# isl-org/Open3D-ML

Hardware: NVIDIA H100
Metric: M points/s forward (higher is better)
Workload: dtype f32

## Files before the change

include/o3dml_b200.h:

```cpp
#ifndef O3DML_B200_H
#define O3DML_B200_H

#include <stddef.h>
#include <stdint.h>

#ifdef __cplusplus
extern "C" {
#endif

#define O3DML_ABI_VERSION 2
#define O3DML_API __attribute__((visibility("default")))

#define O3DML_ACT_NONE 0
#define O3DML_ACT_RELU 1
#define O3DML_ACT_LEAKY 2

O3DML_API int o3dml_abi_version(void);
O3DML_API const char* o3dml_last_error(void);
O3DML_API unsigned long long o3dml_launch_count(void);
O3DML_API void o3dml_launch_count_add(unsigned long long n);


O3DML_API size_t o3dml_voxelize_workspace_bytes(int64_t num_points, int64_t batch);
O3DML_API int o3dml_voxelize(const float* points, int64_t num_points, int point_stride,
// ... 127 lines not shown
                                    const void* weight_image, int k_pad, int n_pad, const float* scale,
                                    const float* shift, int act, float slope, float* out,
                                    int out_channels, void* stream);
O3DML_API int o3dml_deconv_nhwc_tc(const float* in, int batch, int H, int W, int C, int stride,
                                   const void* weight_image, int k_pad, int n_pad, const float* scale,
                                   const float* shift, int act, float slope, float* out, int out_ld,
                                   int out_channels, void* stream);

O3DML_API int o3dml_linear_rows_small_supported(int channels0, int channels1, int out_channels);
O3DML_API int o3dml_linear_rows_small(int64_t num_rows, const o3dml_src_t* srcs, int num_srcs,
                                      const float* h_weight_t, const float* h_scale,
                                      const float* h_shift, int act, float slope, float* out, int out_ld,
                                      int out_channels, void* stream);


O3DML_API int o3dml_randla_lfa_pool(int stage, int d, const float* coords, const void* neighbor_idx,
                          int idx_is64, int num_neighbors, const float* feat, int64_t batch,
                          int64_t n_per_batch, const float* w10_t, const float* s10,
                          const float* t10, const float* wl2_t, const float* s2, const float* t2,
                          const float* wscore_t, const float* bscore, float* agg, void* stream);

#define O3DML_LFA16_WEIGHT_FLOATS 448
O3DML_API int o3dml_randla_lfa16_pool(int stage, const float* coords, const void* neighbor_idx, int idx_is64,
                                      int num_neighbors, const float* feat, int64_t batch,
                                      int64_t n_per_batch, const float* h_weights, float* agg,
                                      void* stream);

O3DML_API int o3dml_randla_lfa_pool_tc(int stage, int d, const float* coords, const void* neighbor_idx,
                                       int idx_is64, int num_neighbors, const float* feat, int64_t batch,
                                       int64_t n_per_batch, const float* w10_t, const float* s10,
                                       const float* t10, const void* wl2_image, const float* wl2_t,
                                       const float* s2, const float* t2, const void* wscore_image,
                                       float* agg, void* stream);

O3DML_API int o3dml_randla_tail_supported(int skip_channels, int coarse_channels, int c1, int c2, int c3, int classes);
O3DML_API int o3dml_randla_tail(const float* skip, int skip_ld, const float* coarse, int coarse_ld,
                                int64_t coarse_rows, const void* interp_index, int index_is64,
                                int64_t out_rows_per_batch, int64_t src_rows_per_batch, int64_t num_rows,
                                const void* weight_image, const float* h_scale, const float* h_shift, float slope,
                                int classes, float* out, void* stream);

O3DML_API int o3dml_gather_max(const float* src, int64_t src_rows, int channels, int src_ld,
                     const void* index, int index_is64, int64_t num_rows, int k,
                     int64_t out_rows_per_batch, int64_t src_rows_per_batch, int shadow_zero,
                     float* out, int out_ld, void* stream);


O3DML_API int o3dml_kpconv_gather(const float* query_points, int64_t num_queries,
                        const float* support_points, int64_t num_support,
                        const void* neighbor_index, int index_is64, int max_neighbors,
                        const float* features, int in_channels, const float* kernel_points,
                        int num_kernel_points, float kp_extent, float* weighted_features,
                        void* stream);

O3DML_API int o3dml_kpconv_gather_deformable(const float* query_points, int64_t num_queries,
                        const float* support_points, int64_t num_support,
                        const void* neighbor_index, int index_is64, int max_neighbors,
                        const float* features, int in_channels, const float* kernel_points,
                        int num_kernel_points, float kp_extent, const float* offsets, int offset_ld,
                        float* weighted_features, void* stream);

#ifdef __cplusplus
}
#endif
#endif
```

open3d-ml_b200/_lib.py:

```python
import ctypes
import math
import os

import torch

_HERE = os.path.dirname(os.path.abspath(__file__))
LIB_PATH = os.path.join(_HERE, "lib", "libo3dml_b200.so")
_lib = None
ABI_VERSION = 2

c_void_p, c_int, c_int64, c_float, c_size_t = (ctypes.c_void_p, ctypes.c_int, ctypes.c_int64,
                                               ctypes.c_float, ctypes.c_size_t)


class Src(ctypes.Structure):
    _fields_ = [("data", c_void_p), ("index", c_void_p), ("rows", c_int64),
                ("out_rows_per_batch", c_int64), ("src_rows_per_batch", c_int64),
                ("channels", ctypes.c_int32), ("ld", ctypes.c_int32),
                ("index_is64", ctypes.c_int32), ("index_ld", ctypes.c_int32)]


P, I, L, F, Z = c_void_p, c_int, c_int64, c_float, c_size_t
_SIGNATURES = {
    "o3dml_abi_version": (c_int, []),
# ... 4 lines not shown
    "o3dml_voxelize": (I, [P, L, I, P, L, P, P, P, L, L, P, P, P, P, P, P, P, Z, P]),
    "o3dml_ragged_to_dense": (I, [P, I, L, P, L, L, L, L, P, P]),
    "o3dml_knn_workspace_bytes": (Z, [L, L, L]),
    "o3dml_knn_search": (I, [P, L, P, P, L, P, L, I, P, I, P, P, Z, P]),
    "o3dml_radius_workspace_bytes": (Z, [L, L, L]),
    "o3dml_radius_count": (I, [P, L, P, P, L, P, L, F, P, P, P, Z, P]),
    "o3dml_radius_fill": (I, [P, L, L, P, L, F, P, P, P, P, Z, P]),
    "o3dml_voxel_reduce": (I, [P, I, P, I, I, P, P, P, P, L, I, I, P, P, P, P]),
    "o3dml_reduce_subarrays_sum": (I, [P, P, L, P, P]),
    "o3dml_sparse_conv_workspace_bytes": (Z, [L]),
    "o3dml_sparse_conv_neighbors": (I, [P, L, P, L, F, P, P, I, P, P, P, Z, P]),
    "o3dml_continuous_conv": (I, [P, I, I, I, I, I, P, L, P, I, P, P, P, L, P, P, I, P, P, I, I, I, I, P, P]),
    "o3dml_nms_workspace_bytes": (Z, [L]),
    "o3dml_nms": (I, [P, P, L, F, P, P, P, Z, P]),
    "o3dml_iou_matrix": (I, [P, L, P, L, I, P, P]),
    "o3dml_pp_detect_workspace_bytes": (Z, [L, L, L, I, I, L]),
    "o3dml_pp_detect": (I, [P, L, P, L, P, L, L, L, L, I, I, P, L, F, F, P, P, P, P, P, Z, P]),
    "o3dml_pp_pfn_scatter": (I, [P, I, I, P, P, P, P, P, L, P, P, P, I, F, F, F, F, I, I, I, P, P,
                                 I, P]),
    "o3dml_pp_pfn2_scatter": (I, [P, I, I, P, P, P, P, P, L, P, P, P, P, P, P, I, F, F, F, F, I, I, I, P, P,
                                  I, P]),
    "o3dml_linear": (I, [L, ctypes.POINTER(Src), I, P, P, P, P, I, I, F, P, I, I, I, P]),
    "o3dml_conv3x3_nhwc": (I, [P, I, I, I, I, I, P, P, P, I, F, P, I, P]),
    "o3dml_deconv_nhwc": (I, [P, I, I, I, I, I, P, P, P, I, F, P, I, I, P]),
    "o3dml_linear_tc_supported": (I, [ctypes.POINTER(Src), I]),
    "o3dml_linear_tc": (I, [L, ctypes.POINTER(Src), I, P, I, I, P, P, P, I, I, F, P, I, I, I, P]),
    "o3dml_conv3x3_nhwc_tc": (I, [P, I, I, I, I, I, P, I, I, P, P, I, F, P, I, P]),
    "o3dml_deconv_nhwc_tc": (I, [P, I, I, I, I, I, P, I, I, P, P, I, F, P, I, I, P]),
    "o3dml_randla_lfa_pool": (I, [I, I, P, P, I, I, P, L, L, P, P, P, P, P, P, P, P, P, P]),
    "o3dml_linear_rows_small_supported": (I, [I, I, I]),
    "o3dml_linear_rows_small": (I, [L, P, I, P, P, P, I, F, P, I, I, P]),
    "o3dml_randla_lfa16_pool": (I, [I, P, P, I, I, P, L, L, P, P, P]),
    "o3dml_randla_lfa_pool_tc": (I, [I, I, P, P, I, I, P, L, L, P, P, P, P, P, P, P, P, P, P]),
    "o3dml_randla_tail_supported": (I, [I, I, I, I, I, I]),
    "o3dml_randla_tail": (I, [P, I, P, I, L, P, I, L, L, L, P, P, P, F, I, P, P]),
    "o3dml_gather_max": (I, [P, L, I, I, P, I, L, I, L, L, I, P, I, P]),
    "o3dml_kpconv_gather": (I, [P, L, P, L, P, I, I, P, I, P, I, F, P, P]),
    "o3dml_kpconv_gather_deformable": (I, [P, L, P, L, P, I, I, P, I, P, I, F, P, I, P, P]),
}
EXPORTS = tuple(_SIGNATURES)
_BRINGUP_SIGNATURES = {
    "o3dml_tc_gemm_test": (I, [P, P, P, I, I, I, P]),
    "o3dml_tc_mma_rate": (I, [I, I, P, P]),
}


def lib():
    global _lib
    if _lib is None:
        from . import build as _build
        have_nvcc = os.path.exists(_build.NVCC)
        if have_nvcc or not os.path.exists(LIB_PATH):
            try:
                _build.build()
            except Exception as e:
                if not os.path.exists(LIB_PATH):
                    raise RuntimeError(
                        "open3d_ml_b200: CUDA library %s is missing and could not be built (%s). "
                        "There is no CPU fallback." % (LIB_PATH, e)) from e
                raise
        h = ctypes.CDLL(LIB_PATH)
        for name, (res, args) in list(_SIGNATURES.items()) + list(_BRINGUP_SIGNATURES.items()):
            fn = getattr(h, name)
            fn.restype, fn.argtypes = res, args
        if h.o3dml_abi_version() != ABI_VERSION:
            raise RuntimeError("open3d_ml_b200: ABI version mismatch")
# ... 235 lines not shown
```

open3d-ml_b200/csrc/common.cuh:

```cuda
#pragma once
#include <cuda_runtime.h>
#include <stdint.h>
#include <stdio.h>
#include <atomic>
#include <utility>

#define O3DML_OK 0
#define O3DML_ERR_INVALID 1
#define O3DML_ERR_WORKSPACE 2
#define O3DML_ERR_CUDA 3
#define O3DML_ERR_UNSUPPORTED 4

extern "C" void o3dml_set_error(const char* fmt, ...);

#define O3DML_FAIL(code, ...)      \
    do {                           \
        o3dml_set_error(__VA_ARGS__); \
        return (code);             \
    } while (0)

#define O3DML_CHECK(cond, ...)                               \
    do {                                                     \
        if (!(cond)) O3DML_FAIL(O3DML_ERR_INVALID, __VA_ARGS__); \
    } while (0)

#define O3DML_CHECK_WORKSPACE(ws, entry)                                                                    \
    do {                                                                                                    \
        if (!(ws).ok) O3DML_FAIL(O3DML_ERR_WORKSPACE, entry ": workspace too small (%zu needed)", (ws).off); \
    } while (0)

#define O3DML_CUDA(...)                                                               \
    do {                                                                              \
        cudaError_t e__ = (__VA_ARGS__);                                              \
        if (e__ != cudaSuccess)                                                       \
            O3DML_FAIL(O3DML_ERR_CUDA, "%s failed: %s (%s:%d)", #__VA_ARGS__,         \
                       cudaGetErrorString(e__), __FILE__, __LINE__);                  \
    } while (0)

namespace o3dml {

constexpr int kNumSMs = 132;

void count_launch();

template <auto Kernel>
cudaError_t opt_in_smem(size_t smem) {
    if (smem <= 48 * 1024) return cudaSuccess;
    static std::atomic<unsigned long long> done{0};
    int dev = -1;
    if (cudaGetDevice(&dev) != cudaSuccess || dev >= 64) dev = -1;
    if (dev >= 0 && ((done.load(std::memory_order_relaxed) >> dev) & 1ull)) return cudaSuccess;
    const cudaError_t e = cudaFuncSetAttribute(Kernel, cudaFuncAttributeMaxDynamicSharedMemorySize, (int)smem);
    if (e == cudaSuccess && dev >= 0) done.fetch_or(1ull << dev, std::memory_order_relaxed);
    return e;
}

template <auto Kernel, class... Args>
cudaError_t launch(dim3 grid, dim3 block, size_t smem, cudaStream_t st, Args&&... args) {
    cudaError_t e = opt_in_smem<Kernel>(smem);
    if (e == cudaSuccess) {
        cudaLaunchConfig_t cfg = {};
        cfg.gridDim = grid;
        cfg.blockDim = block;
        cfg.dynamicSmemBytes = smem;
        cfg.stream = st;
        e = cudaLaunchKernelEx(&cfg, Kernel, std::forward<Args>(args)...);
    }
    if (e != cudaSuccess) {
        cudaGetLastError();
        return e;
    }
    count_launch();
    return cudaSuccess;
}

inline int device_sm_count() {
    int dev = 0, n = 0;
    if (cudaGetDevice(&dev) == cudaSuccess && cudaDeviceGetAttribute(&n, cudaDevAttrMultiProcessorCount, dev) == cudaSuccess &&
        n > 0)
        return n;
    return kNumSMs;
}

template <typename T>
__host__ __device__ inline T ceil_div(T a, T b) {
    return (a + b - 1) / b;
}

struct Workspace {
    char* base;
    size_t size, off = 0;
    bool ok = true;
    Workspace(void* p, size_t n) : base((char*)p), size(n) {}
    template <class Carve, class... Args>
    static size_t measure(Carve carve, Args... args) {
        Workspace ws(nullptr, 0);
        carve(ws, args...);
        return ws.off;
// ... 68 lines not shown
```

open3d-ml_b200/csrc/lfa_tc.cu:

```cuda
#include "../../include/o3dml_b200.h"
#include "common.cuh"
#include "tc.cuh"

namespace o3dml {

constexpr int LTC_ROWS = 128;
constexpr int LTC_K = 16;

struct LfaTcParams {
    const float* coords;
    const void* nidx;
    int nidx_is64;
    const float* feat;
    int64_t total, n_per_batch;
    const float* w10t;
    const float* s10;
    const float* t10;
    const uint4* wl2_img;
    const float* wl2t;
    const float* s2;
    const float* t2;
    const uint4* ws_img;
    float* agg;
    int64_t num_tiles;
};

template <int D, int STAGE>
struct LtcCfg {
    static constexpr int H = D / 2;
    static constexpr bool STREAM = D > 128;
    static constexpr bool MMA2 = STAGE == 2 && H >= 16;
    static constexpr int NTH = 256;
    static constexpr int NPART = NTH / LTC_ROWS;
    static constexpr int CB = D < 64 ? D : (STREAM ? 32 : 64);
    static constexpr int NBLK = D / CB;
    static constexpr int CB2 = STREAM ? 32 : (H < 64 ? H : 64);
    static constexpr int A_BYTES = D / 8 * LTC_ROWS * 16;
    static constexpr int SLOT_BYTES = D / 8 * CB * 16;
    static constexpr int B_BYTES = STREAM ? 2 * SLOT_BYTES : D / 8 * D * 16;
    static constexpr int B2_BYTES = MMA2 ? (STREAM ? H / 8 * CB2 * 16 : H / 8 * H * 16) : 0;
    static constexpr int W10_BYTES = 12 * H * 4;
    static constexpr int ST2_BYTES = STAGE == 2 ? (2 * H + (H < 16 ? H * H : 0)) * 4 : 0;
    static constexpr int MIN_CTAS = D == 64 ? 2 : 1;
    static constexpr bool DBUF = D == 128;
    static constexpr int NBUF = DBUF ? 2 : 1;
    static constexpr size_t SMEM = NBUF * 2 * A_BYTES + 2 * B_BYTES + 2 * B2_BYTES + W10_BYTES + ST2_BYTES + 16 + 128;
};

template <int CBN, int K>
__device__ __forceinline__ void ltc_issue(float* d, uint32_t a_hi, uint32_t a_lo, uint32_t b_hi, uint32_t b_lo,
                                          uint32_t b_lbo, int wg) {
    constexpr uint32_t A_LBO = LTC_ROWS * 16;
    a_hi += (uint32_t)wg * 64 * 16;
    a_lo += (uint32_t)wg * 64 * 16;
#pragma unroll
    for (int i = 0; i < CBN / 2; ++i) tc::fence_operand(d[i]);
    tc::wgmma_fence();
#pragma unroll
    for (int ks = 0; ks < K / 16; ++ks) {
        const uint64_t ah = tc::smem_desc(a_hi + ks * 2 * A_LBO, A_LBO, 128);
        const uint64_t al = tc::smem_desc(a_lo + ks * 2 * A_LBO, A_LBO, 128);
        const uint64_t bh = tc::smem_desc(b_hi + ks * 2 * b_lbo, b_lbo, 128);
        const uint64_t bl = tc::smem_desc(b_lo + ks * 2 * b_lbo, b_lbo, 128);
        tc::wgmma_f16_ss<CBN>(d, ah, bh, ks > 0);
        tc::wgmma_f16_ss<CBN>(d, ah, bl, 1u);
        tc::wgmma_f16_ss<CBN>(d, al, bh, 1u);
    }
    tc::wgmma_commit();
#pragma unroll
    for (int i = 0; i < CBN / 2; ++i) tc::fence_operand(d[i]);
}

template <int N, int CNT>
__device__ __forceinline__ void ltc_wait(float* d) {
    tc::wgmma_wait<N>();
#pragma unroll
    for (int i = 0; i < CNT; ++i) tc::fence_operand(d[i]);
}

template <int CBN, int K, int NIMG>
__device__ __forceinline__ void ltc_fill(uint8_t* slot, uint64_t* bar, const uint4* __restrict__ img, int nb, int lane,
                                         bool issuer) {
    constexpr uint32_t ROW = CBN * 16, HALF = K / 8 * ROW;
    asm volatile("{\n\t.reg .pred p;\n\tsetp.ne.b32 p, %2, 0;\n\t"
                 "@p mbarrier.arrive.expect_tx.shared::cta.b64 _, [%0], %1;\n\t}" ::"r"(tc::smem_u32(bar)),
                 "r"(2 * HALF), "r"((int)(issuer && lane == 0))
                 : "memory");
#pragma unroll
    for (int i0 = 0; i0 < 2 * (K / 8); i0 += 32) {
        const int i = i0 + lane, im = i / (K / 8), kc = i % (K / 8);
        asm volatile("{\n\t.reg .pred p;\n\tsetp.ne.b32 p, %4, 0;\n\t"
                     "@p cp.async.bulk.shared::cluster.global.mbarrier::complete_tx::bytes [%0], [%1], %2, [%3];\n\t}"
                     ::"r"(tc::smem_u32(slot + im * HALF + kc * ROW)),
                     "l"(img + ((size_t)im * (K / 8) + kc) * NIMG + nb * CBN), "r"(ROW), "r"(tc::smem_u32(bar)),
                     "r"((int)(issuer && i < 2 * (K / 8)))
                     : "memory");
    }
}

template <int CNT, int BIT>
__device__ __forceinline__ void ltc_reduce_scatter(float* a, float* b, int lane, int& base) {
    if constexpr (BIT >= 4) {
        if constexpr (CNT > 1) {
            constexpr int h = CNT / 2;
            const bool up = (lane & BIT) != 0;
#pragma unroll
            for (int i = 0; i < h; ++i) {
                const float ra = __shfl_xor_sync(0xffffffffu, up ? a[i] : a[i + h], BIT);
                const float rb = __shfl_xor_sync(0xffffffffu, up ? b[i] : b[i + h], BIT);
                a[i] = (up ? a[i + h] : a[i]) + ra;
                b[i] = (up ? b[i + h] : b[i]) + rb;
            }
            base += up ? h : 0;
            ltc_reduce_scatter<h, BIT / 2>(a, b, lane, base);
        } else {
            a[0] += __shfl_xor_sync(0xffffffffu, a[0], BIT);
            b[0] += __shfl_xor_sync(0xffffffffu, b[0], BIT);
            ltc_reduce_scatter<1, BIT / 2>(a, b, lane, base);
        }
    }
}

template <int D, int STAGE>
__global__ void __launch_bounds__(LtcCfg<D, STAGE>::NTH, LtcCfg<D, STAGE>::MIN_CTAS)
lfa_pool_tc_kernel(const __grid_constant__ LfaTcParams p) {
    using C = LtcCfg<D, STAGE>;
    constexpr int H = C::H, NTH = C::NTH, NPART = C::NPART, CB = C::CB, CB2 = C::CB2;
    extern __shared__ __align__(128) uint8_t smem[];
    uint8_t* b_sm = smem + C::NBUF * 2 * C::A_BYTES;
    uint8_t* b2_sm = b_sm + 2 * C::B_BYTES;
    float* W10 = reinterpret_cast<float*>(b2_sm + 2 * C::B2_BYTES);
    float* ST2 = W10 + 12 * H;
    uint64_t* ring_full = reinterpret_cast<uint64_t*>(reinterpret_cast<uint8_t*>(W10) + C::W10_BYTES + C::ST2_BYTES);

    const int tid = threadIdx.x, lane = tid & 31;
    const int row = tid & (LTC_ROWS - 1);
    const int half = tid >> 7;
    const int wg = tid >> 7, g = lane >> 2, t = lane & 3;
    const int r0 = wg * 64 + ((tid >> 5) & 3) * 16 + g;
    const int pt = r0 >> 4;

    if (!C::STREAM) {
        for (int i = tid; i < 2 * C::B_BYTES / 16; i += NTH)
            reinterpret_cast<uint4*>(b_sm)[i] = p.ws_img[i];
        if (C::MMA2)
            for (int i = tid; i < 2 * C::B2_BYTES / 16; i += NTH)
                reinterpret_cast<uint4*>(b2_sm)[i] = p.wl2_img[i];
    }
    if (STAGE == 2) {
        for (int i = tid; i < H; i += NTH) {
            ST2[i] = p.s2[i];
            ST2[H + i] = p.t2[i];
        }
        if (H < 16)
            for (int i = tid; i < H * H; i += NTH) ST2[2 * H + i] = p.wl2t[i];
    }
    for (int i = tid; i < 10 * H; i += NTH) W10[i] = p.w10t[i];
    for (int i = tid; i < H; i += NTH) {
        W10[10 * H + i] = p.s10[i];
        W10[11 * H + i] = p.t10[i];
    }
    uint32_t ring_phase = 0;
    if (C::STREAM && tid == 0) {
        tc::mbar_init(&ring_full[0], 1);
        tc::mbar_init(&ring_full[1], 1);
        tc::fence_mbar_init();
    }
    tc::fence_async_smem();
    __syncthreads();
    if (C::STREAM) {
        ltc_fill<CB, D, D>(b_sm, &ring_full[0], p.ws_img, 0, lane, tid < 32);
        ltc_fill<CB, D, D>(b_sm + 2 * C::SLOT_BYTES, &ring_full[1], p.ws_img, 1, lane, tid < 32);
    }

    constexpr bool PREF = D >= 64;
    constexpr bool LATE = C::STREAM;
    constexpr bool RAW_INDEX = C::STREAM;
    constexpr int FCH = PREF ? (H / 8) / NPART : 1;
    int64_t g_nx = p.total, nb_nx = -1, g_n2 = p.total, base_n2 = -1;
    RawIndex raw_n2 = {0, 0};
    float qc_nx[6] = {0.f, 0.f, 0.f, 0.f, 0.f, 0.f};
    float4 f_nx[FCH][2];
    auto load_idx = [&](int64_t t, int64_t& g_, int64_t& base_, RawIndex& raw_) {
        g_ = p.total;
        base_ = -1;
        if (t < p.num_tiles) {
            g_ = t * (LTC_ROWS / LTC_K) + (row >> 4);
            if (g_ < p.total) {
                base_ = (g_ / p.n_per_batch) * p.n_per_batch;
                if (RAW_INDEX) load_index_raw(p.nidx, g_ * LTC_K + (row & 15), p.nidx_is64, raw_);
                else base_ += load_index(p.nidx, g_ * LTC_K + (row & 15), p.nidx_is64);
            }
        }
    };
    auto resolve = [&](int64_t base_, const RawIndex& raw_) -> int64_t {
        if (!RAW_INDEX) return base_;
        return base_ >= 0 ? base_ + index_value(raw_, p.nidx_is64) : (int64_t)-1;
    };
    auto load_data = [&](int64_t g_, int64_t nb_, float* qc, float4 (*f)[2]) {
        if (nb_ >= 0) {
            qc[0] = p.coords[3 * g_]; qc[1] = p.coords[3 * g_ + 1]; qc[2] = p.coords[3 * g_ + 2];
            qc[3] = p.coords[3 * nb_]; qc[4] = p.coords[3 * nb_ + 1]; qc[5] = p.coords[3 * nb_ + 2];
#pragma unroll
            for (int i = 0; i < FCH; ++i) {
                const float* src = p.feat + (size_t)nb_ * H + (half + i * NPART) * 8;
                f[i][0] = *reinterpret_cast<const float4*>(src);
                f[i][1] = *reinterpret_cast<const float4*>(src + 4);
            }
        } else {
#pragma unroll
            for (int i = 0; i < 6; ++i) qc[i] = 0.f;
#pragma unroll
            for (int i = 0; i < FCH; ++i) f[i][0] = f[i][1] = make_float4(0.f, 0.f, 0.f, 0.f);
        }
    };
    auto advance = [&](int64_t tile) {
        g_nx = g_n2;
        nb_nx = resolve(base_n2, raw_n2);
        load_data(g_nx, nb_nx, qc_nx, f_nx);
        load_idx(tile + 2 * (int64_t)gridDim.x, g_n2, base_n2, raw_n2);
    };
    if (PREF) {
        load_idx(blockIdx.x, g_nx, base_n2, raw_n2);
        nb_nx = resolve(base_n2, raw_n2);
        load_data(g_nx, nb_nx, qc_nx, f_nx);
        load_idx((int64_t)blockIdx.x + gridDim.x, g_n2, base_n2, raw_n2);
    }

    auto encode = [&](int64_t nb_, const float* qc, float* e) {
#pragma unroll
        for (int q = 0; q < 10; ++q) e[q] = 0.f;
        if (nb_ >= 0) {
            const float dx = qc[0] - qc[3], dy = qc[1] - qc[4], dz = qc[2] - qc[5];
            e[0] = sqrtf(__fadd_rn(__fadd_rn(__fmul_rn(dx, dx), __fmul_rn(dy, dy)), __fmul_rn(dz, dz)));
            e[1] = dx; e[2] = dy; e[3] = dz;
            e[4] = qc[0]; e[5] = qc[1]; e[6] = qc[2];
            e[7] = qc[3]; e[8] = qc[4]; e[9] = qc[5];
        }
    };
    auto locse = [&](const float* e, uint8_t* dst_hi, uint8_t* dst_lo) {
        for (int ch = half; ch < H / 8; ch += NPART) {
            float r[8];
#pragma unroll
            for (int j = 0; j < 8; ++j) r[j] = 0.f;
#pragma unroll
            for (int q = 0; q < 10; ++q) {
                const float4 wa = *reinterpret_cast<const float4*>(&W10[q * H + ch * 8]);
                const float4 wb = *reinterpret_cast<const float4*>(&W10[q * H + ch * 8 + 4]);
                ffma2(r[0], r[1], e[q], wa.x, wa.y);
                ffma2(r[2], r[3], e[q], wa.z, wa.w);
                ffma2(r[4], r[5], e[q], wb.x, wb.y);
                ffma2(r[6], r[7], e[q], wb.z, wb.w);
            }
            {
                const float4 sa = *reinterpret_cast<const float4*>(&W10[10 * H + ch * 8]);
                const float4 sb = *reinterpret_cast<const float4*>(&W10[10 * H + ch * 8 + 4]);
                const float4 ta = *reinterpret_cast<const float4*>(&W10[11 * H + ch * 8]);
                const float4 tb = *reinterpret_cast<const float4*>(&W10[11 * H + ch * 8 + 4]);
                const float sc[8] = {sa.x, sa.y, sa.z, sa.w, sb.x, sb.y, sb.z, sb.w};
                const float sh[8] = {ta.x, ta.y, ta.z, ta.w, tb.x, tb.y, tb.z, tb.w};
#pragma unroll
                for (int j = 0; j < 8; ++j) {
                    const float a = fmaf(r[j], sc[j], sh[j]);
                    r[j] = a >= 0.f ? a : 0.2f * a;
                }
            }
            if (STAGE == 2 && !C::MMA2) {
                float r2[8];
#pragma unroll
                for (int j = 0; j < 8; ++j) {
                    float a = 0.f;
#pragma unroll
                    for (int i = 0; i < 8; ++i) a = fmaf(r[i], ST2[2 * H + i * H + j], a);
                    a = fmaf(a, ST2[j], ST2[H + j]);
                    r2[j] = a >= 0.f ? a : 0.2f * a;
                }
#pragma unroll
                for (int j = 0; j < 8; ++j) r[j] = r2[j];
            }
            uint4 hi, lo;
            tc::split8(r, hi, lo);
            *reinterpret_cast<uint4*>(dst_hi + tc::op_off(LTC_ROWS, row, ch)) = hi;
            *reinterpret_cast<uint4*>(dst_lo + tc::op_off(LTC_ROWS, row, ch)) = lo;
        }
    };
    constexpr uint32_t R1_OFF = (STAGE == 2 && C::MMA2) ? 0u : (uint32_t)(H / 8) * LTC_ROWS * 16;

    auto build = [&](int64_t tile, uint8_t* a_hi, uint8_t* a_lo) {
        int64_t g = tile * (LTC_ROWS / LTC_K) + (row >> 4);
        int64_t nb = -1;
        float4 f_cur[FCH][2];
        if (PREF) {
            g = g_nx;
            nb = nb_nx;
            float qc[6];
#pragma unroll
            for (int i = 0; i < 6; ++i) qc[i] = qc_nx[i];
#pragma unroll
            for (int i = 0; i < FCH; ++i) { f_cur[i][0] = f_nx[i][0]; f_cur[i][1] = f_nx[i][1]; }
            if (!LATE) advance(tile);
            float e[10];
            encode(nb, qc, e);
            locse(e, a_hi + R1_OFF, a_lo + R1_OFF);
        } else {
            float qc[6] = {0.f, 0.f, 0.f, 0.f, 0.f, 0.f};
            if (g < p.total) {
                const int64_t b = g / p.n_per_batch;
                nb = b * p.n_per_batch + load_index(p.nidx, g * LTC_K + (row & 15), p.nidx_is64);
                qc[0] = p.coords[3 * g]; qc[1] = p.coords[3 * g + 1]; qc[2] = p.coords[3 * g + 2];
                qc[3] = p.coords[3 * nb]; qc[4] = p.coords[3 * nb + 1]; qc[5] = p.coords[3 * nb + 2];
            }
            float e[10];
            encode(nb, qc, e);
            locse(e, a_hi + R1_OFF, a_lo + R1_OFF);
        }
        auto store_features = [&]() {
#pragma unroll
            for (int fi = 0; fi < (H / 8 + NPART - 1) / NPART; ++fi) {
                const int ch = half + fi * NPART;
                if (ch >= H / 8) break;
                float x[8];
                if (PREF) {
                    const float4 v0 = f_cur[fi < FCH ? fi : 0][0], v1 = f_cur[fi < FCH ? fi : 0][1];
                    x[0] = v0.x; x[1] = v0.y; x[2] = v0.z; x[3] = v0.w;
                    x[4] = v1.x; x[5] = v1.y; x[6] = v1.z; x[7] = v1.w;
                } else if (nb >= 0) {
                    const float4 v0 = *reinterpret_cast<const float4*>(p.feat + (size_t)nb * H + ch * 8);
                    const float4 v1 = *reinterpret_cast<const float4*>(p.feat + (size_t)nb * H + ch * 8 + 4);
                    x[0] = v0.x; x[1] = v0.y; x[2] = v0.z; x[3] = v0.w;
                    x[4] = v1.x; x[5] = v1.y; x[6] = v1.z; x[7] = v1.w;
                } else {
#pragma unroll
                    for (int j = 0; j < 8; ++j) x[j] = 0.f;
                }
                uint4 hi, lo;
                tc::split8(x, hi, lo);
                *reinterpret_cast<uint4*>(a_hi + tc::op_off(LTC_ROWS, row, ch)) = hi;
                *reinterpret_cast<uint4*>(a_lo + tc::op_off(LTC_ROWS, row, ch)) = lo;
            }
        };

        if (C::MMA2) {
            tc::fence_async_smem();
            __syncthreads();
#pragma unroll 1
            for (int blk = 0; blk < H / CB2; ++blk) {
                if (C::STREAM) {
                    if (blk > 0) __syncthreads();
                    constexpr int N_U4 = H / 8 * CB2;
                    for (int i = tid; i < 2 * N_U4; i += NTH) {
                        const int im = i / N_U4, rem = i % N_U4, kc = rem / CB2, r = rem % CB2;
                        reinterpret_cast<uint4*>(b2_sm + im * C::B2_BYTES)[rem] =
                            p.wl2_img[(size_t)im * (H / 8) * H + kc * H + blk * CB2 + r];
                    }
                    tc::fence_async_smem();
                    __syncthreads();
                }
                const uint32_t bh = tc::smem_u32(b2_sm) + (C::STREAM ? 0u : (uint32_t)blk * CB2 * 16);
                float d2[CB2 / 2];
                ltc_issue<CB2, H>(d2, tc::smem_u32(a_hi), tc::smem_u32(a_lo), bh, bh + C::B2_BYTES,
                                  (C::STREAM ? CB2 : H) * 16, wg);
                ltc_wait<0, CB2 / 2>(d2);
#pragma unroll
                for (int q = 0; q < CB2 / 8; ++q) {
                    const int c = blk * CB2 + 8 * q + 2 * t;
                    const float2 sc = *reinterpret_cast<const float2*>(&ST2[c]);
                    const float2 sh = *reinterpret_cast<const float2*>(&ST2[H + c]);
#pragma unroll
                    for (int hh = 0; hh < 2; ++hh) {
                        float v0 = fmaf(d2[4 * q + 2 * hh], sc.x, sh.x), v1 = fmaf(d2[4 * q + 2 * hh + 1], sc.y, sh.y);
                        v0 = v0 >= 0.f ? v0 : 0.2f * v0;
                        v1 = v1 >= 0.f ? v1 : 0.2f * v1;
                        const uint32_t hi = tc::cvt_f16x2(v0, v1);
                        const float2 f = __half22float2(*reinterpret_cast<const __half2*>(&hi));
                        const uint32_t off = tc::op_off(LTC_ROWS, r0 + 8 * hh, (H + blk * CB2) / 8 + q) + 4 * t;
                        *reinterpret_cast<uint32_t*>(a_hi + off) = hi;
                        *reinterpret_cast<uint32_t*>(a_lo + off) = tc::cvt_f16x2(v0 - f.x, v1 - f.y);
                    }
                }
            }
            __syncthreads();
        }
        store_features();
        if (PREF && LATE) advance(tile);
        tc::fence_async_smem();
    };

    auto softmax = [&](int64_t tile, const float* s, int c0, const uint8_t* a_hi, const uint8_t* a_lo) {
            const int64_t gp = tile * (LTC_ROWS / LTC_K) + pt;
            constexpr int M = CB / 4;
            float den[M], num[M];
#pragma unroll
            for (int q = 0; q < CB / 8; ++q) {
                const uint32_t off = tc::op_off(LTC_ROWS, r0, c0 / 8 + q) + 4 * t;
                const float2 h0 = __half22float2(*reinterpret_cast<const __half2*>(a_hi + off));
                const float2 l0 = __half22float2(*reinterpret_cast<const __half2*>(a_lo + off));
                const float2 h1 = __half22float2(*reinterpret_cast<const __half2*>(a_hi + off + 8 * 16));
                const float2 l1 = __half22float2(*reinterpret_cast<const __half2*>(a_lo + off + 8 * 16));
                const float x0[2] = {h0.x + l0.x, h0.y + l0.y}, x1[2] = {h1.x + l1.x, h1.y + l1.y};
#pragma unroll
                for (int u = 0; u < 2; ++u) {
                    const float v0 = s[4 * q + u], v1 = s[4 * q + 2 + u];
                    float m = fmaxf(v0, v1);
                    m = fmaxf(m, __shfl_xor_sync(0xffffffffu, m, 4));
                    m = fmaxf(m, __shfl_xor_sync(0xffffffffu, m, 8));
                    m = fmaxf(m, __shfl_xor_sync(0xffffffffu, m, 16));
                    const float ml = -m * kLog2e;
                    const float e0 = ex2_ftz(fmaf(v0, kLog2e, ml)), e1 = ex2_ftz(fmaf(v1, kLog2e, ml));
                    den[2 * q + u] = e0 + e1;
                    num[2 * q + u] = e0 * x0[u] + e1 * x1[u];
                }
            }
            int base = 0;
            ltc_reduce_scatter<M, 16>(den, num, lane, base);
            if (gp < p.total) {
                float* dst = p.agg + (size_t)gp * D + c0 + 8 * (base >> 1) + 2 * t;
                if (M == 16) *reinterpret_cast<float2*>(dst) = make_float2(num[0] / den[0], num[1] / den[1]);
                else if (M > 4 || !(lane & 4)) dst[base & 1] = num[0] / den[0];
            }
        };
    auto issue = [&](float* d, int j, uint32_t ah, uint32_t al) {
            if (C::STREAM) {
                const int s = j & 1;
                tc::mbar_wait(&ring_full[s], (ring_phase >> s) & 1u);
                ring_phase ^= 1u << s;
                const uint32_t bh = tc::smem_u32(b_sm) + (uint32_t)s * 2 * C::SLOT_BYTES;
                ltc_issue<CB, D>(d, ah, al, bh, bh + C::SLOT_BYTES, CB * 16, wg);
            } else {
                const uint32_t bh = tc::smem_u32(b_sm) + (uint32_t)j * CB * 16;
                ltc_issue<CB, D>(d, ah, al, bh, bh + C::B_BYTES, D * 16, wg);
            }
        };
    float acc0[CB / 2], acc1[CB / 2];
    if (C::DBUF) {
        static_assert(!C::DBUF || (C::NBLK == 2 && !C::STREAM), "double-buffered A: two resident score blocks");
        build(blockIdx.x, smem, smem + C::A_BYTES);
        __syncthreads();
        int buf = 0;
#pragma unroll 1
        for (int64_t tile = blockIdx.x; tile < p.num_tiles; tile += gridDim.x) {
            uint8_t* a_hi = smem + buf * 2 * C::A_BYTES;
            uint8_t* nx_hi = smem + (buf ^ 1) * 2 * C::A_BYTES;
            const uint32_t ah = tc::smem_u32(a_hi), al = ah + C::A_BYTES;
            issue(acc0, 0, ah, al);
            issue(acc1, 1, ah, al);
            build(tile + gridDim.x, nx_hi, nx_hi + C::A_BYTES);
            ltc_wait<1, CB / 2>(acc0);
            softmax(tile, acc0, 0, a_hi, a_hi + C::A_BYTES);
            ltc_wait<0, CB / 2>(acc1);
            softmax(tile, acc1, CB, a_hi, a_hi + C::A_BYTES);
            __syncthreads();
            buf ^= 1;
        }
        return;
    }
    uint8_t* a_hi = smem;
    uint8_t* a_lo = smem + C::A_BYTES;
    const uint32_t ah = tc::smem_u32(a_hi), al = tc::smem_u32(a_lo);
    for (int64_t tile = blockIdx.x; tile < p.num_tiles; tile += gridDim.x) {
        build(tile, a_hi, a_lo);
        __syncthreads();
        const bool more = tile + gridDim.x < p.num_tiles;
        auto step = [&](int j, float* cur, float* nxt) {
            if (j + 1 < C::NBLK) {
                issue(nxt, j + 1, ah, al);
                ltc_wait<1, CB / 2>(cur);
            } else {
                ltc_wait<0, CB / 2>(cur);
            }
            if (C::STREAM) {
                __syncthreads();
                ltc_fill<CB, D, D>(b_sm + (j & 1) * 2 * C::SLOT_BYTES, &ring_full[j & 1], p.ws_img,
                                   j + 2 < C::NBLK ? j + 2 : j + 2 - C::NBLK, lane, tid < 32 && (j + 2 < C::NBLK || more));
            }
            softmax(tile, cur, j * CB, a_hi, a_lo);
        };
        issue(acc0, 0, ah, al);
        if (C::NBLK == 1) {
            step(0, acc0, acc1);
        } else {
#pragma unroll 1
            for (int j = 0; j < C::NBLK; j += 2) {
                step(j, acc0, acc1);
                step(j + 1, acc1, acc0);
            }
        }
        __syncthreads();
    }
}

template <int D, int STAGE>
static int lfa_tc_launch(const LfaTcParams& p, cudaStream_t st) {
    using C = LtcCfg<D, STAGE>;
    static_assert(C::SMEM <= 227 * 1024, "shared memory budget");
    O3DML_CUDA(opt_in_smem<lfa_pool_tc_kernel<D, STAGE>>(C::SMEM));
    int per_sm = 0;
    O3DML_CUDA(cudaOccupancyMaxActiveBlocksPerMultiprocessor(&per_sm, lfa_pool_tc_kernel<D, STAGE>, C::NTH, C::SMEM));
    if (per_sm < 1) per_sm = 1;
    if (per_sm > 4) per_sm = 4;
    int64_t grid = (int64_t)device_sm_count() * per_sm;
    if (grid > p.num_tiles) grid = p.num_tiles;
    O3DML_CUDA(launch<lfa_pool_tc_kernel<D, STAGE>>((unsigned)grid, C::NTH, C::SMEM, st, p));
    return O3DML_OK;
}

}

using namespace o3dml;

extern "C" int o3dml_randla_lfa_pool_tc(int stage, int d, const float* coords, const void* neighbor_idx,
                                        int idx_is64, int num_neighbors, const float* feat, int64_t batch,
                                        int64_t n_per_batch, const float* w10_t, const float* s10,
                                        const float* t10, const void* wl2_image, const float* wl2_t,
                                        const float* s2, const float* t2, const void* wscore_image,
                                        float* agg, void* stream) {
    O3DML_CHECK(stage == 1 || stage == 2, "lfa_tc: stage must be 1 or 2");
    O3DML_CHECK(num_neighbors == LTC_K, "lfa_tc: built for 16 neighbours");
    O3DML_CHECK(batch * n_per_batch < ((int64_t)1 << 31), "lfa_tc: too many points");
    O3DML_CHECK(stage == 1 || (s2 && t2 && (d == 16 ? wl2_t != nullptr : wl2_image != nullptr)),
                "lfa_tc: stage 2 needs the lse2 weights");
    LfaTcParams p;
    p.coords = coords; p.nidx = neighbor_idx; p.nidx_is64 = idx_is64; p.feat = feat;
    p.total = batch * n_per_batch; p.n_per_batch = n_per_batch;
    p.w10t = w10_t; p.s10 = s10; p.t10 = t10;
    p.wl2_img = (const uint4*)wl2_image; p.wl2t = wl2_t; p.s2 = s2; p.t2 = t2;
    p.ws_img = (const uint4*)wscore_image; p.agg = agg;
    p.num_tiles = ceil_div<int64_t>(p.total, LTC_ROWS / LTC_K);
    if (p.total == 0) return O3DML_OK;
    cudaStream_t st = (cudaStream_t)stream;
#define LTC_CASE(DD) \
    case DD: return stage == 1 ? lfa_tc_launch<DD, 1>(p, st) : lfa_tc_launch<DD, 2>(p, st);
    switch (d) {
        LTC_CASE(16)
        LTC_CASE(32)
        LTC_CASE(64)
        LTC_CASE(128)
        LTC_CASE(256)
        default:
            O3DML_FAIL(O3DML_ERR_UNSUPPORTED, "lfa_tc: d_out %d not in {16,32,64,128,256}", d);
    }
#undef LTC_CASE
}
```

open3d-ml_b200/csrc/tc.cuh:

```cuda
#pragma once
#include <cuda_fp16.h>
#include <cuda_runtime.h>
#include <stdint.h>

namespace o3dml {
namespace tc {

__device__ __forceinline__ uint32_t smem_u32(const void* p) {
    return static_cast<uint32_t>(__cvta_generic_to_shared(p));
}

__device__ __forceinline__ void mbar_init(uint64_t* bar, uint32_t count) {
    asm volatile("mbarrier.init.shared::cta.b64 [%0], %1;" ::"r"(smem_u32(bar)), "r"(count));
}
__device__ __forceinline__ void fence_mbar_init() {
    asm volatile("fence.mbarrier_init.release.cluster;" ::: "memory");
}
__device__ __forceinline__ void mbar_wait(uint64_t* bar, uint32_t parity) {
    asm volatile(
        "{\n\t.reg .pred p;\n\t"
        "WAIT_%=:\n\t"
        "mbarrier.try_wait.parity.shared::cta.b64 p, [%0], %1;\n\t"
        "@p bra DONE_%=;\n\t"
        "bra WAIT_%=;\n\t"
        "DONE_%=:\n\t}" ::"r"(smem_u32(bar)), "r"(parity)
        : "memory");
}

__device__ __forceinline__ void bulk_copy_g2s(void* smem_dst, const void* gsrc, uint32_t bytes, uint64_t* bar) {
    asm volatile("cp.async.bulk.shared::cluster.global.mbarrier::complete_tx::bytes [%0], [%1], %2, [%3];" ::"r"(
                     smem_u32(smem_dst)),
                 "l"(gsrc), "r"(bytes), "r"(smem_u32(bar))
                 : "memory");
}
__device__ __forceinline__ void mbar_arrive_expect_tx(uint64_t* bar, uint32_t bytes) {
    asm volatile("mbarrier.arrive.expect_tx.shared::cta.b64 _, [%0], %1;" ::"r"(smem_u32(bar)), "r"(bytes) : "memory");
}

__device__ __forceinline__ void fence_async_smem() {
    asm volatile("fence.proxy.async.shared::cta;" ::: "memory");
}
__device__ __forceinline__ uint64_t smem_desc(uint32_t saddr, uint32_t lbo_bytes, uint32_t sbo_bytes) {
    uint64_t d = 0;
    d |= (uint64_t)((saddr >> 4) & 0x3fffu);
    d |= (uint64_t)((lbo_bytes >> 4) & 0x3fffu) << 16;
    d |= (uint64_t)((sbo_bytes >> 4) & 0x3fffu) << 32;
    return d;
}
__device__ __forceinline__ uint64_t smem_desc_sw128(uint32_t saddr) {
    return (uint64_t)((saddr >> 4) & 0x3fffu) | ((uint64_t)1 << 16) | ((uint64_t)(1024 >> 4) << 32) | ((uint64_t)1 << 62);
}
__device__ __forceinline__ void wgmma_fence() { asm volatile("wgmma.fence.sync.aligned;" ::: "memory"); }
__device__ __forceinline__ void wgmma_commit() { asm volatile("wgmma.commit_group.sync.aligned;" ::: "memory"); }
__device__ __forceinline__ void wgmma_wait_all() { asm volatile("wgmma.wait_group.sync.aligned 0;" ::: "memory"); }

__device__ __forceinline__ void split_tf32(uint32_t x, uint32_t& hi, uint32_t& lo) {
    hi = x & 0xFFFFE000u;
    lo = __float_as_uint(__uint_as_float(x) - __uint_as_float(hi));
}

template <int N> __device__ void wgmma_tf32_rs(float* d, const uint32_t* a, uint64_t bdesc, uint32_t scale_d);
template <> __device__ __forceinline__ void wgmma_tf32_rs<32>(float* d, const uint32_t* a, uint64_t bdesc, uint32_t scale_d) {
    asm volatile(
        "{\n\t.reg .pred p;\n\tsetp.ne.b32 p, %21, 0;\n\t"
        "wgmma.mma_async.sync.aligned.m64n32k8.f32.tf32.tf32 {%0, %1, %2, %3, %4, %5, %6, %7, %8, %9, %10, %11, %12, %13, %14, %15}, {%16, %17, %18, %19}, %20, p, 1, 1;\n\t}"
        : "+f"(d[0]), "+f"(d[1]), "+f"(d[2]), "+f"(d[3]), "+f"(d[4]), "+f"(d[5]), "+f"(d[6]), "+f"(d[7]), "+f"(d[8]), "+f"(d[9]), "+f"(d[10]), "+f"(d[11]), "+f"(d[12]), "+f"(d[13]), "+f"(d[14]), "+f"(d[15])
        : "r"(a[0]), "r"(a[1]), "r"(a[2]), "r"(a[3]), "l"(bdesc), "r"(scale_d)
        : "memory");
}
template <> __device__ __forceinline__ void wgmma_tf32_rs<64>(float* d, const uint32_t* a, uint64_t bdesc, uint32_t scale_d) {
    asm volatile(
        "{\n\t.reg .pred p;\n\tsetp.ne.b32 p, %37, 0;\n\t"
        "wgmma.mma_async.sync.aligned.m64n64k8.f32.tf32.tf32 {%0, %1, %2, %3, %4, %5, %6, %7, %8, %9, %10, %11, %12, %13, %14, %15, %16, %17, %18, %19, %20, %21, %22, %23, %24, %25, %26, %27, %28, %29, %30, %31}, {%32, %33, %34, %35}, %36, p, 1, 1;\n\t}"
// ... 70 lines not shown
```

Baseline: 141.8.

## Split d=256 stage-1 LFA score GEMM across 4-CTA thread block clusters

For d_out=256 stage 1, the score weights no longer stream through a double-buffered ring. Each tile is now processed by a cluster of 4 CTAs, each holding a resident quarter of the weight columns. Each CTA builds a quarter of the A rows and broadcasts them to its peers through distributed shared memory stores, synchronising with cluster barriers. This removes the weight streaming and ring synchronisation, at the cost of DSMEM traffic, cluster barrier latency, and fewer concurrent tiles. A concurrency query export is also added.

```diff
diff --git a/include/o3dml_b200.h b/include/o3dml_b200.h
--- a/include/o3dml_b200.h
+++ b/include/o3dml_b200.h
@@ -183,6 +183,7 @@
                                        const float* t10, const void* wl2_image, const float* wl2_t,
                                        const float* s2, const float* t2, const void* wscore_image,
                                        float* agg, void* stream);
+O3DML_API int o3dml_randla_lfa_pool_tc_concurrency(int stage, int d, int* tiles);
 
 O3DML_API int o3dml_randla_tail_supported(int skip_channels, int coarse_channels, int c1, int c2, int c3, int classes);
 O3DML_API int o3dml_randla_tail(const float* skip, int skip_ld, const float* coarse, int coarse_ld,
diff --git a/open3d-ml_b200/_lib.py b/open3d-ml_b200/_lib.py
--- a/open3d-ml_b200/_lib.py
+++ b/open3d-ml_b200/_lib.py
@@ -60,6 +60,7 @@
     "o3dml_linear_rows_small": (I, [L, P, I, P, P, P, I, F, P, I, I, P]),
     "o3dml_randla_lfa16_pool": (I, [I, P, P, I, I, P, L, L, P, P, P]),
     "o3dml_randla_lfa_pool_tc": (I, [I, I, P, P, I, I, P, L, L, P, P, P, P, P, P, P, P, P, P]),
+    "o3dml_randla_lfa_pool_tc_concurrency": (I, [I, I, ctypes.POINTER(ctypes.c_int)]),
     "o3dml_randla_tail_supported": (I, [I, I, I, I, I, I]),
     "o3dml_randla_tail": (I, [P, I, P, I, L, P, I, L, L, L, P, P, P, F, I, P, P]),
     "o3dml_gather_max": (I, [P, L, I, I, P, I, L, I, L, L, I, P, I, P]),
diff --git a/open3d-ml_b200/csrc/common.cuh b/open3d-ml_b200/csrc/common.cuh
--- a/open3d-ml_b200/csrc/common.cuh
+++ b/open3d-ml_b200/csrc/common.cuh
@@ -55,7 +55,7 @@
     return e;
 }
 
-template <auto Kernel, class... Args>
+template <auto Kernel, unsigned Cluster = 1, class... Args>
 cudaError_t launch(dim3 grid, dim3 block, size_t smem, cudaStream_t st, Args&&... args) {
     cudaError_t e = opt_in_smem<Kernel>(smem);
     if (e == cudaSuccess) {
@@ -64,6 +64,15 @@
         cfg.blockDim = block;
         cfg.dynamicSmemBytes = smem;
         cfg.stream = st;
+        cudaLaunchAttribute attr = {};
+        if (Cluster > 1) {
+            attr.id = cudaLaunchAttributeClusterDimension;
+            attr.val.clusterDim.x = Cluster;
+            attr.val.clusterDim.y = 1;
+            attr.val.clusterDim.z = 1;
+            cfg.attrs = &attr;
+            cfg.numAttrs = 1;
+        }
         e = cudaLaunchKernelEx(&cfg, Kernel, std::forward<Args>(args)...);
     }
     if (e != cudaSuccess) {
diff --git a/open3d-ml_b200/csrc/lfa_tc.cu b/open3d-ml_b200/csrc/lfa_tc.cu
--- a/open3d-ml_b200/csrc/lfa_tc.cu
+++ b/open3d-ml_b200/csrc/lfa_tc.cu
@@ -28,16 +28,19 @@
 template <int D, int STAGE>
 struct LtcCfg {
     static constexpr int H = D / 2;
-    static constexpr bool STREAM = D > 128;
+    static constexpr bool CLUSTER = D > 128 && STAGE == 1;
+    static constexpr bool STREAM = D > 128 && !CLUSTER;
+    static constexpr int CL = CLUSTER ? 4 : 1;
+    static constexpr int BROWS = LTC_ROWS / CL;
     static constexpr bool MMA2 = STAGE == 2 && H >= 16;
     static constexpr int NTH = 256;
-    static constexpr int NPART = NTH / LTC_ROWS;
+    static constexpr int NPART = NTH / BROWS;
     static constexpr int CB = D < 64 ? D : (STREAM ? 32 : 64);
-    static constexpr int NBLK = D / CB;
+    static constexpr int NBLK = D / CL / CB;
     static constexpr int CB2 = STREAM ? 32 : (H < 64 ? H : 64);
     static constexpr int A_BYTES = D / 8 * LTC_ROWS * 16;
     static constexpr int SLOT_BYTES = D / 8 * CB * 16;
-    static constexpr int B_BYTES = STREAM ? 2 * SLOT_BYTES : D / 8 * D * 16;
+    static constexpr int B_BYTES = STREAM ? 2 * SLOT_BYTES : D / 8 * (D / CL) * 16;
     static constexpr int B2_BYTES = MMA2 ? (STREAM ? H / 8 * CB2 * 16 : H / 8 * H * 16) : 0;
     static constexpr int W10_BYTES = 12 * H * 4;
     static constexpr int ST2_BYTES = STAGE == 2 ? (2 * H + (H < 16 ? H * H : 0)) * 4 : 0;
@@ -96,6 +99,12 @@
                      "r"((int)(issuer && i < 2 * (K / 8)))
                      : "memory");
     }
+}
+
+template <int N, int K, int NIMG, int NTH>
+__device__ __forceinline__ void ltc_load_cols(uint8_t* dst, const uint4* __restrict__ img, int c0, int tid) {
+    for (int i = tid; i < 2 * (K / 8) * N; i += NTH)
+        reinterpret_cast<uint4*>(dst)[i] = img[(size_t)(i / N) * NIMG + c0 + i % N];
 }
 
 template <int CNT, int BIT>
@@ -134,13 +143,18 @@
     uint64_t* ring_full = reinterpret_cast<uint64_t*>(reinterpret_cast<uint8_t*>(W10) + C::W10_BYTES + C::ST2_BYTES);
 
     const int tid = threadIdx.x, lane = tid & 31;
-    const int row = tid & (LTC_ROWS - 1);
-    const int half = tid >> 7;
+    const int crank = C::CLUSTER ? (int)tc::cluster_ctarank() : 0;
+    const unsigned first = C::CLUSTER ? tc::cluster_id() : blockIdx.x;
+    const unsigned stride = C::CLUSTER ? tc::cluster_count() : gridDim.x;
+    const int row = C::CLUSTER ? crank * C::BROWS + (tid & (C::BROWS - 1)) : tid & (LTC_ROWS - 1);
+    const int half = C::CLUSTER ? tid / C::BROWS : tid >> 7;
     const int wg = tid >> 7, g = lane >> 2, t = lane & 3;
     const int r0 = wg * 64 + ((tid >> 5) & 3) * 16 + g;
     const int pt = r0 >> 4;
 
-    if (!C::STREAM) {
+    if constexpr (C::CLUSTER) {
+        ltc_load_cols<D / C::CL, D, D, NTH>(b_sm, p.ws_img, crank * (D / C::CL), tid);
+    } else if (!C::STREAM) {
         for (int i = tid; i < 2 * C::B_BYTES / 16; i += NTH)
             reinterpret_cast<uint4*>(b_sm)[i] = p.ws_img[i];
         if (C::MMA2)
@@ -167,15 +181,22 @@
         tc::fence_mbar_init();
     }
     tc::fence_async_smem();
-    __syncthreads();
+    if constexpr (C::CLUSTER) {
+        tc::cluster_arrive_relaxed();
+    } else {
+        __syncthreads();
+    }
+    uint32_t peer[C::CL];
+#pragma unroll
+    for (int r = 0; r < C::CL; ++r) peer[r] = C::CLUSTER ? tc::mapa(tc::smem_u32(smem), (crank + r) % C::CL) : 0u;
     if (C::STREAM) {
         ltc_fill<CB, D, D>(b_sm, &ring_full[0], p.ws_img, 0, lane, tid < 32);
         ltc_fill<CB, D, D>(b_sm + 2 * C::SLOT_BYTES, &ring_full[1], p.ws_img, 1, lane, tid < 32);
     }
 
     constexpr bool PREF = D >= 64;
-    constexpr bool LATE = C::STREAM;
-    constexpr bool RAW_INDEX = C::STREAM;
+    constexpr bool LATE = D > 128;
+    constexpr bool RAW_INDEX = D > 128;
     constexpr int FCH = PREF ? (H / 8) / NPART : 1;
     int64_t g_nx = p.total, nb_nx = -1, g_n2 = p.total, base_n2 = -1;
     RawIndex raw_n2 = {0, 0};
@@ -218,13 +239,13 @@
         g_nx = g_n2;
         nb_nx = resolve(base_n2, raw_n2);
         load_data(g_nx, nb_nx, qc_nx, f_nx);
-        load_idx(tile + 2 * (int64_t)gridDim.x, g_n2, base_n2, raw_n2);
+        load_idx(tile + 2 * (int64_t)stride, g_n2, base_n2, raw_n2);
     };
     if (PREF) {
-        load_idx(blockIdx.x, g_nx, base_n2, raw_n2);
+        load_idx(first, g_nx, base_n2, raw_n2);
         nb_nx = resolve(base_n2, raw_n2);
         load_data(g_nx, nb_nx, qc_nx, f_nx);
-        load_idx((int64_t)blockIdx.x + gridDim.x, g_n2, base_n2, raw_n2);
+        load_idx((int64_t)first + stride, g_n2, base_n2, raw_n2);
     }
 
     auto encode = [&](int64_t nb_, const float* qc, float* e) {
@@ -238,6 +259,18 @@
             e[7] = qc[3]; e[8] = qc[4]; e[9] = qc[5];
         }
     };
+    auto put = [&](uint8_t* dst_hi, uint8_t* dst_lo, uint32_t off, const uint4& hi, const uint4& lo) {
+        *reinterpret_cast<uint4*>(dst_hi + off) = hi;
+        *reinterpret_cast<uint4*>(dst_lo + off) = lo;
+        if constexpr (C::CLUSTER) {
+            const uint32_t oh = (uint32_t)(dst_hi - smem) + off, ol = (uint32_t)(dst_lo - smem) + off;
+#pragma unroll
+            for (int r = 1; r < C::CL; ++r) {
+                tc::st_cluster(peer[r] + oh, hi);
+                tc::st_cluster(peer[r] + ol, lo);
+            }
+        }
+    };
     auto locse = [&](const float* e, uint8_t* dst_hi, uint8_t* dst_lo) {
         for (int ch = half; ch < H / 8; ch += NPART) {
             float r[8];
@@ -280,8 +313,7 @@
             }
             uint4 hi, lo;
             tc::split8(r, hi, lo);
-            *reinterpret_cast<uint4*>(dst_hi + tc::op_off(LTC_ROWS, row, ch)) = hi;
-            *reinterpret_cast<uint4*>(dst_lo + tc::op_off(LTC_ROWS, row, ch)) = lo;
+            put(dst_hi, dst_lo, tc::op_off(LTC_ROWS, row, ch), hi, lo);
         }
     };
     constexpr uint32_t R1_OFF = (STAGE == 2 && C::MMA2) ? 0u : (uint32_t)(H / 8) * LTC_ROWS * 16;
@@ -301,6 +333,7 @@
             if (!LATE) advance(tile);
             float e[10];
             encode(nb, qc, e);
+            if constexpr (C::CLUSTER) tc::cluster_wait();
             locse(e, a_hi + R1_OFF, a_lo + R1_OFF);
         } else {
             float qc[6] = {0.f, 0.f, 0.f, 0.f, 0.f, 0.f};
@@ -335,8 +368,7 @@
                 }
                 uint4 hi, lo;
                 tc::split8(x, hi, lo);
-                *reinterpret_cast<uint4*>(a_hi + tc::op_off(LTC_ROWS, row, ch)) = hi;
-                *reinterpret_cast<uint4*>(a_lo + tc::op_off(LTC_ROWS, row, ch)) = lo;
+                put(a_hi, a_lo, tc::op_off(LTC_ROWS, row, ch), hi, lo);
             }
         };
 
@@ -382,8 +414,9 @@
             __syncthreads();
         }
         store_features();
-        if (PREF && LATE) advance(tile);
-        tc::fence_async_smem();
+        if (PREF && LATE && !C::CLUSTER) advance(tile);
+        if constexpr (C::CLUSTER) tc::fence_async_smem_cluster();
+        else tc::fence_async_smem();
     };
 
     auto softmax = [&](int64_t tile, const float* s, int c0, const uint8_t* a_hi, const uint8_t* a_lo) {
@@ -428,7 +461,7 @@
                 ltc_issue<CB, D>(d, ah, al, bh, bh + C::SLOT_BYTES, CB * 16, wg);
             } else {
                 const uint32_t bh = tc::smem_u32(b_sm) + (uint32_t)j * CB * 16;
-                ltc_issue<CB, D>(d, ah, al, bh, bh + C::B_BYTES, D * 16, wg);
+                ltc_issue<CB, D>(d, ah, al, bh, bh + C::B_BYTES, (D / C::CL) * 16, wg);
             }
         };
     float acc0[CB / 2], acc1[CB / 2];
@@ -457,50 +490,94 @@
     uint8_t* a_hi = smem;
     uint8_t* a_lo = smem + C::A_BYTES;
     const uint32_t ah = tc::smem_u32(a_hi), al = tc::smem_u32(a_lo);
-    for (int64_t tile = blockIdx.x; tile < p.num_tiles; tile += gridDim.x) {
-        build(tile, a_hi, a_lo);
-        __syncthreads();
-        const bool more = tile + gridDim.x < p.num_tiles;
-        auto step = [&](int j, float* cur, float* nxt) {
-            if (j + 1 < C::NBLK) {
-                issue(nxt, j + 1, ah, al);
-                ltc_wait<1, CB / 2>(cur);
+    if constexpr (C::CLUSTER) {
+        static_assert(C::NBLK == 1 && PREF && !C::MMA2, "clusters: one score block per CTA, stage 1");
+#pragma unroll 1
+        for (int64_t tile = first; tile < p.num_tiles; tile += stride) {
+            build(tile, a_hi, a_lo);
+            tc::cluster_sync();
+            tc::fence_async_smem();
+            if (LATE) advance(tile);
+            issue(acc0, 0, ah, al);
+            ltc_wait<0, CB / 2>(acc0);
+            softmax(tile, acc0, crank * CB, a_hi, a_lo);
+            tc::cluster_arrive_relaxed();
+        }
+        tc::cluster_wait();
+    } else {
+        for (int64_t tile = blockIdx.x; tile < p.num_tiles; tile += gridDim.x) {
+            build(tile, a_hi, a_lo);
+            __syncthreads();
+            const bool more = tile + gridDim.x < p.num_tiles;
+            auto step = [&](int j, float* cur, float* nxt) {
+                if (j + 1 < C::NBLK) {
+                    issue(nxt, j + 1, ah, al);
+                    ltc_wait<1, CB / 2>(cur);
+                } else {
+                    ltc_wait<0, CB / 2>(cur);
+                }
+                if (C::STREAM) {
+                    __syncthreads();
+                    ltc_fill<CB, D, D>(b_sm + (j & 1) * 2 * C::SLOT_BYTES, &ring_full[j & 1], p.ws_img,
+                                       j + 2 < C::NBLK ? j + 2 : j + 2 - C::NBLK, lane,
+                                       tid < 32 && (j + 2 < C::NBLK || more));
+                }
+                softmax(tile, cur, j * CB, a_hi, a_lo);
+            };
+            issue(acc0, 0, ah, al);
+            if (C::NBLK == 1) {
+                step(0, acc0, acc1);
             } else {
-                ltc_wait<0, CB / 2>(cur);
-            }
-            if (C::STREAM) {
-                __syncthreads();
-                ltc_fill<CB, D, D>(b_sm + (j & 1) * 2 * C::SLOT_BYTES, &ring_full[j & 1], p.ws_img,
-                                   j + 2 < C::NBLK ? j + 2 : j + 2 - C::NBLK, lane, tid < 32 && (j + 2 < C::NBLK || more));
-            }
-            softmax(tile, cur, j * CB, a_hi, a_lo);
-        };
-        issue(acc0, 0, ah, al);
-        if (C::NBLK == 1) {
-            step(0, acc0, acc1);
-        } else {
 #pragma unroll 1
-            for (int j = 0; j < C::NBLK; j += 2) {
-                step(j, acc0, acc1);
-                step(j + 1, acc1, acc0);
-            }
-        }
-        __syncthreads();
-    }
+                for (int j = 0; j < C::NBLK; j += 2) {
+                    step(j, acc0, acc1);
+                    step(j + 1, acc1, acc0);
+                }
+            }
+            __syncthreads();
+        }
+    }
+}
+
+template <int D, int STAGE>
+static int lfa_tc_units(int& units) {
+    using C = LtcCfg<D, STAGE>;
+    static_assert(C::SMEM <= 227 * 1024, "shared memory budget");
+    O3DML_CUDA(opt_in_smem<lfa_pool_tc_kernel<D, STAGE>>(C::SMEM));
+    if constexpr (C::CLUSTER) {
+        cudaLaunchConfig_t cfg = {};
+        cudaLaunchAttribute attr = {};
+        attr.id = cudaLaunchAttributeClusterDimension;
+        attr.val.clusterDim.x = C::CL;
+        attr.val.clusterDim.y = 1;
+        attr.val.clusterDim.z = 1;
+        cfg.gridDim = dim3(C::CL);
+        cfg.blockDim = dim3(C::NTH);
+        cfg.dynamicSmemBytes = C::SMEM;
+        cfg.attrs = &attr;
+        cfg.numAttrs = 1;
+        O3DML_CUDA(cudaOccupancyMaxActiveClusters(&units, lfa_pool_tc_kernel<D, STAGE>, &cfg));
+        if (units < 1)
+            O3DML_FAIL(O3DML_ERR_UNSUPPORTED, "lfa_tc: no cluster of %d CTAs with %d KB of shared memory each fits "
+                       "on this device (d = %d)", C::CL, (int)(C::SMEM / 1024), D);
+    } else {
+        int per_sm = 0;
+        O3DML_CUDA(cudaOccupancyMaxActiveBlocksPerMultiprocessor(&per_sm, lfa_pool_tc_kernel<D, STAGE>, C::NTH, C::SMEM));
+        if (per_sm < 1) per_sm = 1;
+        if (per_sm > 4) per_sm = 4;
+        units = device_sm_count() * per_sm;
+    }
+    return O3DML_OK;
 }
 
 template <int D, int STAGE>
 static int lfa_tc_launch(const LfaTcParams& p, cudaStream_t st) {
     using C = LtcCfg<D, STAGE>;
-    static_assert(C::SMEM <= 227 * 1024, "shared memory budget");
-    O3DML_CUDA(opt_in_smem<lfa_pool_tc_kernel<D, STAGE>>(C::SMEM));
-    int per_sm = 0;
-    O3DML_CUDA(cudaOccupancyMaxActiveBlocksPerMultiprocessor(&per_sm, lfa_pool_tc_kernel<D, STAGE>, C::NTH, C::SMEM));
-    if (per_sm < 1) per_sm = 1;
-    if (per_sm > 4) per_sm = 4;
-    int64_t grid = (int64_t)device_sm_count() * per_sm;
-    if (grid > p.num_tiles) grid = p.num_tiles;
-    O3DML_CUDA(launch<lfa_pool_tc_kernel<D, STAGE>>((unsigned)grid, C::NTH, C::SMEM, st, p));
+    int units = 0;
+    const int rc = lfa_tc_units<D, STAGE>(units);
+    if (rc != O3DML_OK) return rc;
+    const int64_t grid = units < p.num_tiles ? units : p.num_tiles;
+    O3DML_CUDA(launch<lfa_pool_tc_kernel<D, STAGE>, C::CL>((unsigned)(grid * C::CL), C::NTH, C::SMEM, st, p));
     return O3DML_OK;
 }
 
@@ -541,3 +618,20 @@
     }
 #undef LTC_CASE
 }
+
+extern "C" int o3dml_randla_lfa_pool_tc_concurrency(int stage, int d, int* tiles) {
+    O3DML_CHECK(stage == 1 || stage == 2, "lfa_tc: stage must be 1 or 2");
+    O3DML_CHECK(tiles != nullptr, "lfa_tc: null output");
+#define LTC_CASE(DD) \
+    case DD: return stage == 1 ? lfa_tc_units<DD, 1>(*tiles) : lfa_tc_units<DD, 2>(*tiles);
+    switch (d) {
+        LTC_CASE(16)
+        LTC_CASE(32)
+        LTC_CASE(64)
+        LTC_CASE(128)
+        LTC_CASE(256)
+        default:
+            O3DML_FAIL(O3DML_ERR_UNSUPPORTED, "lfa_tc: d_out %d not in {16,32,64,128,256}", d);
+    }
+#undef LTC_CASE
+}
diff --git a/open3d-ml_b200/csrc/tc.cuh b/open3d-ml_b200/csrc/tc.cuh
--- a/open3d-ml_b200/csrc/tc.cuh
+++ b/open3d-ml_b200/csrc/tc.cuh
@@ -39,6 +39,48 @@
 
 __device__ __forceinline__ void fence_async_smem() {
     asm volatile("fence.proxy.async.shared::cta;" ::: "memory");
+}
+
+__device__ __forceinline__ uint32_t cluster_ctarank() {
+    uint32_t r;
+    asm volatile("mov.u32 %0, %%cluster_ctarank;" : "=r"(r));
+    return r;
+}
+__device__ __forceinline__ uint32_t cluster_id() {
+    uint32_t r;
+    asm volatile("mov.u32 %0, %%clusterid.x;" : "=r"(r));
+    return r;
+}
+__device__ __forceinline__ uint32_t cluster_count() {
+    uint32_t r;
+    asm volatile("mov.u32 %0, %%nclusterid.x;" : "=r"(r));
+    return r;
+}
+__device__ __forceinline__ uint32_t mapa(uint32_t saddr, uint32_t rank) {
+    uint32_t r;
+    asm volatile("mapa.shared::cluster.u32 %0, %1, %2;" : "=r"(r) : "r"(saddr), "r"(rank));
+    return r;
+}
+__device__ __forceinline__ void st_cluster(uint32_t caddr, const uint4& v) {
+    asm volatile("st.shared::cluster.v4.b32 [%0], {%1, %2, %3, %4};" ::"r"(caddr), "r"(v.x), "r"(v.y), "r"(v.z),
+                 "r"(v.w)
+                 : "memory");
+}
+__device__ __forceinline__ void fence_async_smem_cluster() {
+    asm volatile("fence.proxy.async.shared::cluster;" ::: "memory");
+}
+__device__ __forceinline__ void cluster_arrive() {
+    asm volatile("barrier.cluster.arrive.release.aligned;" ::: "memory");
+}
+__device__ __forceinline__ void cluster_arrive_relaxed() {
+    asm volatile("barrier.cluster.arrive.relaxed.aligned;" ::: "memory");
+}
+__device__ __forceinline__ void cluster_wait() {
+    asm volatile("barrier.cluster.wait.acquire.aligned;" ::: "memory");
+}
+__device__ __forceinline__ void cluster_sync() {
+    cluster_arrive();
+    cluster_wait();
 }
 __device__ __forceinline__ uint64_t smem_desc(uint32_t saddr, uint32_t lbo_bytes, uint32_t sbo_bytes) {
     uint64_t d = 0;
```

Result: no change. 142.2, median of 6 (+0.3%).
